# urbste/pyTheiaSfM

Measured on AMD Instinct MI355X. Metric: BA residuals/sec (LM-iterations/sec x observations); RANSAC hypotheses/sec alongside, higher is better.
Workload: dtype f64; 1 GPU; synth_ba_v1 C4: 1000 views / 500000 tracks / 3001239 observations, mixed pinhole + double-sphere (8 intrinsics groups), TRIVIAL loss, intrinsics NONE, homogeneous-manifold points, 8 LM iterations per solve, use_inner_iterations = false on the GPU and the CPU leg (the trust-region step of north_star alone; the reference's default = true is measured in "with_inner_iterations"); views=1000, tracks=500000, observations=3001239, reduced_system_n=6000, k3_levels=8, fused_kernel_runs=2102, n_ranks_seen_by_rccl=1, n_ranks_in_process_group=1

## Files before the change

### pytheiasfm_amd/csrc/ba_fused.hip

```cpp
#define THIP_LEAN_SQRT 1
#define THIP_LEAN_SINCOS 1
#include "ba_fused_lin.h"

#include <algorithm>
#include <cstdio>
#include <cstdlib>

namespace thip {
namespace {

constexpr int kRowBytes = 24;
static_assert(kFusedMaxCams <= kRowBytes, "slot-table row too short");

__global__ __launch_bounds__(256) void k_cam_prep(DevProblem P, const double* __restrict__ cam, const double* __restrict__ intr,
                                                  double* __restrict__ camrot, const double* __restrict__ ycam) {
  const int c = blockIdx.x * blockDim.x + threadIdx.x;
  if (c == 0 && P.frun_next) { P.frun_next[0] = 0; P.frun_next[1] = 0; }
  if (c >= P.nc) return;
  cam_prep_one(P, c, cam + 6 * (size_t)c, intr, camrot);
  if (ycam && P.camdir) {
    const int rc = P.cam_red[c];
    const unsigned mask = P.cam_mask[c];
    double dl[6], ext[6], out[12];
    for (int q = 0; q < 6; ++q)
// ... 199 lines not shown
    double eh[2 * PD];
#pragma unroll
    for (int i = 0; i < 2; ++i)
#pragma unroll
      for (int b = 0; b < PD; ++b) {
        double sm = 0.0;
#pragma unroll
        for (int k = 0; k <= b; ++k) sm += Jt[i * PD + k] * Li[b][k];
        eh[i * PD + b] = sm;
      }
    double2* Rr = reinterpret_cast<double2*>(s_rec + slot * RD);
#pragma unroll
    for (int k = 0; k < 6; ++k) Rr[k] = make_double2(Jc[2 * k], Jc[2 * k + 1]);
#pragma unroll
    for (int k = 0; k < PD; ++k) Rr[6 + k] = make_double2(eh[2 * k], eh[2 * k + 1]);
    Rr[6 + PD] = make_double2(r[0], r[1]);
    double v1[2];
#pragma unroll
    for (int i = 0; i < 2; ++i) {
      double sm = 0.0;
#pragma unroll
      for (int b = 0; b < PD; ++b) sm += eh[i * PD + b] * gh[b];
      v1[i] = r[i] - sm;
    }
    Rr[6 + PD + 1] = make_double2(v1[0], v1[1]);
    s_tslot[c.tl * kRowBytes + c.lc] = (uint8_t)slot;
  }
  sl.lap(stamps, 5);
  const double costw = wave_sum_all(cost);
  gmax = wave_max_all(gmax);
  const double inval = wave_count(active && !valid);
  const double npd = wave_count(active && !pd_ok && sg.head);
  if (lane == 0 && tile_ok) {
    tile_part[4 * (size_t)tile + 0] = costw;
    tile_part[4 * (size_t)tile + 1] = gmax;
    tile_part[4 * (size_t)tile + 2] = inval;
    tile_part[4 * (size_t)tile + 3] = npd;
  }
  sl.lap(stamps, 6);
}

template <int PD, int TPS, unsigned MODELS, int LOSSK, bool STAMPS = false, bool FIRST = false>
__global__ __launch_bounds__(64 * TPS, THIP_FUSED_WAVES) void k_lin_schur(DevProblem P, const double* __restrict__ pts,
                                                           const double* __restrict__ radius_p,
                                                           double* __restrict__ Vinv, double* __restrict__ tile_part,
                                                           double* __restrict__ scale_out = nullptr) {
  constexpr int RD = rec_doubles<PD>();
  constexpr int SUB = TPS * kWave;
  constexpr int SUBT = TPS * kFusedTileTracks;
  constexpr int NWV = TPS;
  __shared__ __attribute__((aligned(16))) double s_rec[SUB * RD];
  __shared__ __attribute__((aligned(16))) double s_cam[kFusedMaxStage * kCamLds];
  __shared__ uint8_t s_tslot[SUBT * kRowBytes];
  __shared__ unsigned s_tmask[SUBT];
  static_assert(SUB * 18 <= SUB * RD, "slice-combination scratch does not fit the record buffer");
  const int tid = threadIdx.x, lane = tid & 63, wv = __builtin_amdgcn_readfirstlane(tid >> 6);
  const double radius = *radius_p;
  const double inv_radius = 1.0 / radius;
  __shared__ int s_next;
  unsigned long long stamps[12];
#pragma unroll
  for (int k = 0; k < 12; ++k) stamps[k] = 0;
  Stamp<STAMPS> sk;
  sk.start();
  int pending = 0;
  if (tid == 0) pending = atomicAdd(P.frun_next, 1);
  for (;;) {
  __syncthreads();
  if (tid == 0) s_next = pending;
  __syncthreads();
  const int rix = __builtin_amdgcn_readfirstlane(s_next);
  if (rix >= P.n_fruns) break;
  if (tid == 0) pending = atomicAdd(P.frun_next, 1);
  const FusedRun run = P.fruns[P.frun_order[rix]];
  const int nsc = (run.ntiles + TPS - 1) / TPS;
  for (int j = tid; j < run.nstage * (kCamRot / 2); j += SUB) {
    const int k = j / (kCamRot / 2), piece = j - k * (kCamRot / 2);
    const int cidx = P.frun_stage[run.stage_off + k];
    reinterpret_cast<double2*>(s_cam + k * kCamLds)[piece] = reinterpret_cast<const double2*>(P.camrot + (size_t)kCamRot * cidx)[piece];
  }
  LanePre<PD> cur;
  int tile = 0; bool tile_ok = false;
  pre_level1<PD, TPS>(P, run, 0, wv, lane, tile, tile_ok, cur);
  pre_level2<PD>(P, pts, cur);
  __syncthreads();

  const int G = run.gp & 0xff, PS = run.gp >> 8;
  int tix, t0, tstride;
  bool slice_ok = true;
  const int B = 64 / PS;
  if (G == 1) { const int g = lane / B; tix = lane - g * B; slice_ok = g < PS; t0 = wv * PS + g; tstride = NWV * PS; }
  else { tix = (wv % G) * 64 + lane; t0 = wv / G; tstride = NWV / G; }
  const bool has_tgt = slice_ok && tix < run.ntgt;
  int la = 0, lb = 0;
  if (has_tgt) { const unsigned us = P.frun_tgt[run.tgt_off + tix]; la = us & 0xffu; lb = us >> 8; }
  const int dix = (G == 1) ? lane : tix;
  const bool has_d = dix < 6 * run.W;
  const int dlc = has_d ? dix / 6 : 0, da = dix % 6;
  const int dP = (G == 1) ? PS : 1, dbase = (G == 1) ? wv * PS : wv / G;
  const unsigned tbits = has_tgt ? ((1u << la) | (1u << lb)) : 0xffffffffu;
  const unsigned dbit = has_d ? (1u << dlc) : 0x80000000u;
  const double diag_core = (has_tgt && la == lb) ? 1.0 : 0.0;
  double acc[36], dacc[3];
#pragma unroll
  for (int k = 0; k < 36; ++k) acc[k] = 0.0;
#pragma unroll
  for (int k = 0; k < 3; ++k) dacc[k] = 0.0;

  sk.lap(stamps, 0);
  for (int sc = 0; sc < nsc; ++sc) {
    LanePre<PD> nxt;
    int ntile = 0; bool ntile_ok = false;
    const int scn = min(sc + 1, nsc - 1);
    pre_level1<PD, TPS>(P, run, scn, wv, lane, ntile, ntile_ok, nxt);
    if (P.fused_dbg & 16) __builtin_amdgcn_s_setprio(1);
    fused_phase_l5<PD, MODELS, LOSSK, STAMPS, FIRST>(P, cur, s_cam, run.W, tile, tile_ok, wv, lane, inv_radius, Vinv, tile_part, s_rec, s_tslot, s_tmask, stamps, scale_out);
    sk.lap(stamps, 1);
    pre_level2<PD>(P, pts, nxt);
    if (P.fused_dbg & 16) __builtin_amdgcn_s_setprio(0);
    if (!(P.fused_dbg & 32)) __builtin_amdgcn_s_setprio(1);
    __syncthreads();
    sk.lap(stamps, 7);
    if (!(P.fused_dbg & 1)) {
      const int last_tile = min(run.tile0 + TPS * sc + TPS - 1, run.tile0 + run.ntiles - 1);
      const int ntr = P.tile_trk_end[last_tile];
      fused_phase_s<PD, RD>(s_rec, s_tslot, s_tmask, ntr, tstride, t0, slice_ok, tbits, la, lb, diag_core, dP, dbase, dbit, dlc, da, acc, dacc);
    }
    sk.lap(stamps, 8);
    if (!(P.fused_dbg & 32)) __builtin_amdgcn_s_setprio(0);
    __syncthreads();
    sk.lap(stamps, 9);
    if constexpr (STAMPS) stamps[11] += 1;
    cur = nxt; tile = ntile; tile_ok = ntile_ok;
  }
  double* scratch = s_rec;
  double* out = P.fpart + run.part_off;
  const int nrep = (G == 1) ? NWV * PS : NWV / G;
#pragma unroll
  for (int h = 0; h < 2; ++h) {
    if (h) __syncthreads();
#pragma unroll
    for (int q = 0; q < 18; ++q) scratch[tid * 18 + q] = acc[18 * h + q];
    __syncthreads();
    for (int e = tid; e < run.ntgt * 18; e += SUB) {
      const int k = e / 18, q = e - 18 * k;
      double v = scratch[k * 18 + q];
#pragma unroll 1
      for (int r = 1; r < nrep; ++r) {
        const int oth = (G == 1) ? ((r / PS) * 64 + (r % PS) * B + k) : (k + r * G * 64);
        v += scratch[oth * 18 + q];
      }
      out[(size_t)k * 36 + 18 * h + q] = v;
    }
  }
  __syncthreads();
#pragma unroll
  for (int q = 0; q < 3; ++q) scratch[tid * 3 + q] = dacc[q];
  __syncthreads();
  if (has_d && tid == dix) {
    const int nrd = (G == 1) ? NWV : NWV / G;
    double v[3];
#pragma unroll
    for (int q = 0; q < 3; ++q) v[q] = scratch[tid * 3 + q];
#pragma unroll 1
    for (int r = 1; r < nrd; ++r) {
      const int oth = (G == 1) ? (r * 64 + dix) : (dix + r * G * 64);
#pragma unroll
      for (int q = 0; q < 3; ++q) v[q] += scratch[oth * 3 + q];
    }
    double* od = out + (size_t)run.ntgt * 36 + (size_t)dix * 3;
#pragma unroll
    for (int q = 0; q < 3; ++q) od[q] = v[q];
  }
  sk.lap(stamps, 10);
  }
  if constexpr (STAMPS) {
    if (lane == 0) {
#pragma unroll
      for (int k = 0; k < 12; ++k) atomicAdd(&g_fused_stamps[k], stamps[k]);
    }
  }
}

constexpr int kCamLdsB = 70;

constexpr int kCamLdsBI = 82;
template <int PD, int TPS, unsigned MODELS, int LOSSK, int WPS, bool INTR = false, unsigned KMASK = 0u>
__global__ __launch_bounds__(64 * TPS, WPS) void k_backsub_runs(DevProblem P, const double* __restrict__ pts, double* __restrict__ cand_pts,
                                                             const double* __restrict__ Vinv, double* __restrict__ tile_part,
                                                             const double* __restrict__ ysol = nullptr) {
  constexpr int NT = PD * (PD + 1) / 2;
  constexpr int SUB = TPS * kWave;
  constexpr int PITCH = INTR ? kCamLdsBI : kCamLdsB;
  constexpr int OFF_CAND = INTR ? 56 : 52;
  constexpr int OFF_CINTR = INTR ? 72 : kCamRotIntr;
  __shared__ __attribute__((aligned(16))) double s_cam[(INTR ? kFusedMaxStageIntr : kFusedMaxStage) * PITCH];
  __shared__ __attribute__((aligned(16))) double s_slot[TPS][64 * 4];
  __shared__ int s_next;
  const int tid = threadIdx.x, lane = tid & 63, wv = __builtin_amdgcn_readfirstlane(tid >> 6);
  int pending = 0;
  if (tid == 0) pending = atomicAdd(P.frun_next + 1, 1);
  for (;;) {
  __syncthreads();
// ... 443 lines not shown
```

### pytheiasfm_amd/csrc/ba_kernels.h

```cpp
#pragma once
#include <algorithm>
#include <vector>
#include <hip/hip_runtime.h>
#include <cstdint>

#include "dense_cholesky.h"

namespace thip {

struct FusedRun {
  int tile0, ntiles;
  int cam_off, W;
  int tgt_off, ntgt;
  int part_off;
  int gp;
  int stage_off, nstage;
};
inline int fused_tiles_per_subchunk(int) { return 4; }
constexpr int kFusedMaxCams = 22;
constexpr int kFusedMaxConst = 22;
constexpr int kFusedMaxStage = kFusedMaxCams + kFusedMaxConst;
constexpr int kFusedTileTracks = 32;
constexpr int kFusedIntrRows = 4, kFusedIntrWidth = 6 + kFusedIntrRows;
constexpr int kFusedMaxCamsIntr = 12;
constexpr int kFusedMaxConstIntr = 12;
constexpr int kFusedMaxStageIntr = kFusedMaxCamsIntr + kFusedMaxConstIntr;

struct DevProblem {
  int nc, np, ncv, ntiles;
  int64_t nobs;
  int n;
  int pd;
  int loss_type;
  double loss_width;
  const double* intr;
  const int* group_model;
  const int* cam_group;
  const int* cam_red;
  const uint8_t* cam_mask;
  const uint8_t* pt_const;
  const double2* obs_uv;
  const double2* obs_si;
  const int* obs_cam;
  const int* obs_pt;
  const int* tile_start;
  const int* tile_count;
  int long_nobs, long_ntracks;
  const int* long_obs_index;
  const int* long_obs_slot;
  const int* long_track_start;
  const int* long_track_pt;
  const double* scale_c;
  const double* scale_p;
  int ni;
  int ng_total;
  const int* grp_k;
  const int* grp_red;
  const unsigned* grp_free;
  const unsigned* red_free;
// ... 228 lines not shown
```

### pytheiasfm_amd/csrc/ba_plan.hip

```cpp
#include <atomic>
#include <cstdio>
#include <limits>
#include <map>
#include <mutex>
#include <new>

#include "ba_handle.h"
#include "ba_host_rules.h"

namespace {

template <class T>
struct NoInitAlloc : std::allocator<T> {
  template <class U> struct rebind { using other = NoInitAlloc<U>; };
  template <class U, class... A>
  void construct(U* ptr, A&&... args) {
    if constexpr (sizeof...(A) == 0) ::new (static_cast<void*>(ptr)) U; else ::new (static_cast<void*>(ptr)) U(std::forward<A>(args)...);
  }
};

template <class T>
struct RawArray {
  std::unique_ptr<T[]> p;
  explicit RawArray(size_t n) : p(new T[std::max<size_t>(1, n)]) {}
  T& operator[](size_t i) { return p[i]; }
  const T& operator[](size_t i) const { return p[i]; }
  T* data() { return p.get(); }
};

template <class T, class Digit>
void counting_pass(const T* from, T* to, int64_t n, int nb, Digit&& digit) {
  int parts = host_part_count(n, 32768);
  if (n < 393216 && !getenv("THEIA_HIP_HOST_CHUNK_MIN")) parts = 1;
  if ((int64_t)parts * nb > ((int64_t)1 << 24)) parts = 1;
  const int64_t per = (n + parts - 1) / parts;
  std::vector<int> head((size_t)parts * nb, 0);
  host_parts(parts, true, [&](int t) {
    int* hh = head.data() + (size_t)t * nb;
    for (int64_t i = t * per; i < std::min<int64_t>(n, (t + 1) * per); ++i) hh[digit(from[i])]++;
  });
  int run = 0;
  for (int b = 0; b < nb; ++b)
    for (int t = 0; t < parts; ++t) { int& c = head[(size_t)t * nb + b]; const int cnt = c; c = run; run += cnt; }
  host_parts(parts, true, [&](int t) {
    int* hh = head.data() + (size_t)t * nb;
    for (int64_t i = t * per; i < std::min<int64_t>(n, (t + 1) * per); ++i) to[hh[digit(from[i])]++] = from[i];
  });
}

__global__ void k_fill_value(double* x, size_t n, double v) {
  for (size_t i = (size_t)blockIdx.x * blockDim.x + threadIdx.x; i < n; i += (size_t)gridDim.x * blockDim.x) x[i] = v;
}

const int kCfgF2S[3][8] = {{SC_COST, SC_GMAX, SC_INVALID, SC_NOTPD, 0, 0, 0, 0},
                           {SB_COST, SB_MCC, SB_STEPSQ, SB_XNORMSQ, SB_INVALID, 0, 0, 0},
                           {SB_COST, SB_INVALID, 0, 0, 0, 0, 0, 0}};
const int kCfgMax[3][8] = {{0, 1, 0, 0, 0, 0, 0, 0}, {0, 0, 0, 0, 0, 0, 0, 0}, {0, 0, 0, 0, 0, 0, 0, 0}};

#define UP(buf, vec) do { rc = h->buf.upload(vec, st); if (rc) return rc; } while (0)
#define AL(buf, cnt) do { rc = h->buf.alloc(cnt); if (rc) return rc; } while (0)
int build_gather_lists(theia_ba_handle_s* h, const int* ocam, const int* opt,
// ... 331 lines not shown
  const bool compact = h->intr_rows == 4;
  emit_pairs(gg, [&](int ga, int gb, int64_t beg, int64_t end) {
    push_item(IT_GG0, 10 * ga, 10 * gb, beg, end, 1 | (ga == gb ? 2 : 0));
    if (!compact) push_item(IT_GG1, 10 * ga, 10 * gb, beg, end, 1 | (ga == gb ? 2 : 0));
  });
  itick("sorted pair lists");
  if (npairs > (size_t)std::numeric_limits<int>::max() - 64)
    return set_error(THEIA_HIP_ERR_UNSUPPORTED, "too many observation pairs for 32-bit pair lists");
  for (size_t q = 0; q < order.size();) {
    size_t e = q + 1;
    while (e < order.size() && red[order[e]] == red[order[q]] && grd[order[e]] == grd[order[q]]) ++e;
    const int rc = red[order[q]], gr = grd[order[q]];
    if (rc >= 0) {
      push_item(IT_CD, h->ni + 6 * rc, h->ni + 6 * rc, (int64_t)q, (int64_t)e, self[rc] ? 1 : 0);
      if (gr >= 0) push_item(IT_CGD, h->ni + 6 * rc, 10 * gr, (int64_t)q, (int64_t)e, 1);
    }
    q = e;
  }
  for (size_t q = 0; q < order.size();) {
    size_t e = q + 1;
    while (e < order.size() && grd[order[e]] == grd[order[q]]) ++e;
    const int gr = grd[order[q]];
    if (gr >= 0) {
      push_item(IT_GD0, 10 * gr, 10 * gr, (int64_t)q, (int64_t)e, 1);
      if (!compact) push_item(IT_GD1, 10 * gr, 10 * gr, (int64_t)q, (int64_t)e, 1);
      push_item(IT_GV, 10 * gr, 10 * gr, (int64_t)q, (int64_t)e, 0);
    }
    q = e;
  }
  h->n_diag_items = 0; h->n_blk_items = (int)items.size() / 6;
  {
    std::vector<int> sobs(order.begin(), order.end());
    if (sobs.empty()) sobs.push_back(0);
    UP(slot_obs, sobs);
  }
  UP(cam_obs, slot); UP(blk_items, items);
  if ((rc = h->blk_pairs.upload(pairs.data(), std::max<size_t>(1, npairs), st, pairs.pinned()))) return rc;
  itick("items + uploads");
  h->n_trk_sums = nsums;
  h->sum_base = nslots;
  if (nsums) { UP(pt_sum_slot, pt_sum); UP(slot_in_sum, slot_sum); UP(pt_sum_cnt, pt_cnt); UP(sum_group, sum_group); }
  AL(rec, (std::max<size_t>(1, order.size()) + (size_t)h->n_trk_sums) * (12 * h->pd + 20 + 2 * h->intr_rows * h->pd + 3 * h->intr_rows));
  return 0;
}

inline int fused_run_cameras(int bw) {
  if (bw == 0) return kFusedMaxCams;
  if (bw == 9) return kFusedMaxCamsIntr;
  if (bw == 10) return 10;
  return 10;
}
inline int fused_lanes_per_target(int bw) { return bw == 0 ? 1 : (bw <= 10 ? (bw + 2) / 3 : (bw + 3) / 4); }

struct FusedHost {
  std::vector<FusedRun> runs;
  std::vector<int> cams, stage, tile_trk_end, sum_items, sum_src;
  std::vector<unsigned short> tgts;
  std::vector<uint8_t> obs_lc, obs_tl;
  std::vector<uint8_t> tile_adj;
  size_t part_doubles = 0;
};
struct FusedSegment {
  std::vector<int> tstart, tcount, tkey, l_obs, l_slot, l_start, l_pt;
  FusedHost fp;
};
void build_fused_segment(const theia_ba_handle_s* h, const std::vector<int64_t>& off, const std::vector<int>& porder,
                         const int* sred, const int* ocam, const std::vector<int>& skey, int q_begin, int q_end,
                         uint8_t* obs_lc, uint8_t* obs_tl, FusedSegment& seg) {
  std::vector<int>& tstart = seg.tstart; std::vector<int>& tcount = seg.tcount; std::vector<int>& tkey = seg.tkey;
  std::vector<int>& l_obs = seg.l_obs; std::vector<int>& l_slot = seg.l_slot; std::vector<int>& l_start = seg.l_start;
  std::vector<int>& l_pt = seg.l_pt;
  FusedHost& fp = seg.fp;
  const int64_t nm = h->nobs_main;
  const int tps = fused_tiles_per_subchunk(h->pd);
  const int bw = h->fused_bw;
  const size_t lanes_tgt = bw == 0 ? 1 : (size_t)fused_lanes_per_target(bw), rows_cam = bw == 0 ? 6 : (size_t)bw;
  const size_t part_tgt = bw == 0 ? 36 : (size_t)bw * bw, part_cam = bw == 0 ? 18 : (size_t)3 * bw;
  const int max_cams = fused_run_cameras(bw);
  const size_t max_tgts = bw == 0 ? 253 : 256 / lanes_tgt;
  auto packing = [&](size_t ntgt, size_t W) -> int {
    if (lanes_tgt * ntgt > 64 || rows_cam * W > 64) return 0;
    static const int cand[6] = {10, 6, 4, 3, 2, 1};
    for (int c : cand) if ((size_t)(64 / c) >= lanes_tgt * ntgt) return c;
    return 1;
  };
  const char* rm = getenv("THEIA_HIP_FUSED_RUN_OBS");
  const int64_t run_max = rm ? std::max(64, atoi(rm)) : std::max<int64_t>(256, std::min<int64_t>(2048, nm / 600));
  int64_t t_start = 0, t_len = 0;
  int t_tracks = 0, sc_tracks = 0;
  int run_tile0 = 0, run_ntiles = 0, run_key0 = -1;
  int64_t run_obs = 0;
  std::vector<int> run_cams;
  std::vector<int64_t> run_pairs;
  std::vector<int> tc;
  std::vector<int64_t> tp;
  int serial = 1, prev_serial = 0;
  std::vector<int> prev_tc;
  std::vector<int> cam_stamp((size_t)std::max(1, h->ncp), 0);
  std::vector<uint8_t> cam_local((size_t)std::max(1, h->ncp), 0);
  const int max_const = bw == 0 ? kFusedMaxConst : kFusedMaxConstIntr;
  static_assert(kFusedMaxConst <= 0x7f && kFusedMaxConstIntr <= 0x7f, "obs_lc keeps the constant-camera index in seven bits");
  std::vector<int> run_ccams, tcc;
  std::vector<int> ccam_stamp((size_t)std::max(1, h->nc), 0);
  std::vector<uint8_t> ccam_local((size_t)std::max(1, h->nc), 0);
  constexpr int kPairSlots = 2048;
  std::vector<int64_t> pair_key(kPairSlots, 0);
  std::vector<int> pair_stamp(kPairSlots, 0);
  auto pair_slot = [&](int64_t key) -> int {
    unsigned hsh = ((unsigned)(key >> 32) * 0x9E3779B1u) ^ ((unsigned)key * 0x85EBCA77u);
    int sl = (int)(hsh >> 21) & (kPairSlots - 1);
    while (pair_stamp[sl] == serial && pair_key[sl] != key) sl = (sl + 1) & (kPairSlots - 1);
    return sl;
  };
  const int adj_nt = (h->n + 63) / 64;
  fp.tile_adj.assign((size_t)adj_nt * adj_nt, 0);
  std::vector<int> tl;
  auto mark_tiles = [&](int q) {
    if (h->pt_const[porder[q]]) return;
    tl.clear();
    for (int pcam : tc) {
      const int rcam = h->cam_red[h->part_cam[pcam]];
      if (rcam < 0) continue;
      const int s0 = h->ni + 6 * rcam;
      if (tl.empty() || tl.back() != s0 / 64) tl.push_back(s0 / 64);
      if ((s0 + 5) / 64 != s0 / 64) tl.push_back((s0 + 5) / 64);
    }
    for (int a : tl) for (int b : tl) fp.tile_adj[(size_t)a * adj_nt + b] = 1;
  };

  auto close_tile = [&](int q_end) {
    if (!t_len) return;
    tstart.push_back((int)t_start); tcount.push_back((int)t_len); tkey.push_back(run_key0 < 0 ? 0 : run_key0);
    (void)q_end;
    fp.tile_trk_end.push_back(sc_tracks);
    run_ntiles++;
    t_len = 0; t_tracks = 0;
  };
  auto finalize_run = [&]() {
    if (!run_ntiles) { run_cams.clear(); run_pairs.clear(); run_ccams.clear(); run_obs = 0; run_key0 = -1; ++serial; return; }
    std::sort(run_cams.begin(), run_cams.end());
    std::sort(run_pairs.begin(), run_pairs.end());
    FusedRun r;
    r.tile0 = run_tile0; r.ntiles = run_ntiles;
    r.cam_off = (int)fp.cams.size(); r.W = (int)run_cams.size();
    fp.cams.insert(fp.cams.end(), run_cams.begin(), run_cams.end());
    r.tgt_off = (int)fp.tgts.size(); r.ntgt = (int)run_pairs.size();
    for (size_t i = 0; i < run_cams.size(); ++i) cam_local[run_cams[i]] = (uint8_t)i;
    for (int64_t key : run_pairs) {
      const int la = cam_local[(int)(key >> 32)], lb = cam_local[(int)(key & 0xffffffff)];
      fp.tgts.push_back((unsigned short)(la | (lb << 8)));
    }
    const int need = (int)std::max(lanes_tgt * r.ntgt, rows_cam * r.W);
    const int G = need <= 64 ? 1 : (need <= 128 ? 2 : 4);
    r.gp = G | ((G == 1 ? std::max(1, packing((size_t)r.ntgt, (size_t)r.W)) : 1) << 8);
    r.part_off = (int)fp.part_doubles;
    fp.part_doubles += (size_t)r.ntgt * part_tgt + (size_t)r.W * part_cam;
    r.stage_off = (int)fp.stage.size();
    for (int pc : run_cams) fp.stage.push_back(h->part_cam[pc]);
    fp.stage.insert(fp.stage.end(), run_ccams.begin(), run_ccams.end());
    r.nstage = (int)(run_cams.size() + run_ccams.size());
    for (int t = run_tile0; t < run_tile0 + run_ntiles; ++t)
      for (int s = tstart[t]; s < tstart[t] + tcount[t]; ++s) {
        if (sred[s] >= 0) obs_lc[s] = cam_local[sred[s]];
        else obs_lc[s] = (uint8_t)(0x80 | ccam_local[ocam[s]]);
      }
    fp.runs.push_back(r);
    run_tile0 += run_ntiles; run_ntiles = 0; run_obs = 0; run_key0 = -1;
    run_cams.clear(); run_pairs.clear(); run_ccams.clear(); ++serial;
  };
  auto push_long = [&](int q) {
    const int slot = (int)l_pt.size();
    l_pt.push_back(porder[q]);
    for (int64_t c = off[q]; c < off[q + 1]; ++c) { l_obs.push_back((int)c); l_slot.push_back(slot); }
    l_start.push_back((int)l_obs.size());
  };
  run_tile0 = (int)tstart.size();
  for (int q = q_begin; q < q_end; ++q) {
    const int64_t L = off[q + 1] - off[q];
    if (L == 0) continue;
    tc.clear(); tcc.clear();
    for (int64_t s = off[q]; s < off[q + 1]; ++s) {
      if (sred[s] >= 0) tc.push_back(sred[s]);
      else tcc.push_back(ocam[s]);
    }
    std::sort(tc.begin(), tc.end());
    const bool dup = std::adjacent_find(tc.begin(), tc.end()) != tc.end();
    if (!tcc.empty()) { std::sort(tcc.begin(), tcc.end()); tcc.erase(std::unique(tcc.begin(), tcc.end()), tcc.end()); }
    mark_tiles(q);
    if (L > 64 || dup || (int)tc.size() > max_cams || (int)tcc.size() > max_const) {
      close_tile(q);
      push_long(q);
      continue;
    }
    const bool same_set = serial == prev_serial && tc == prev_tc;
    size_t ucams = run_cams.size(), upairs = run_pairs.size();
    if (!same_set) {
      tp.clear();
      for (size_t a = 0; a < tc.size(); ++a)
        for (size_t b = 0; b <= a; ++b) tp.push_back(((int64_t)tc[a] << 32) | (uint32_t)tc[b]);
      for (int c : tc) ucams += cam_stamp[c] != serial;
      for (int64_t key : tp) upairs += pair_stamp[pair_slot(key)] != serial;
    }
    bool new_run = (int)ucams > max_cams || upairs > max_tgts;
    if (!tcc.empty()) {
      size_t uc = run_ccams.size();
      for (int c : tcc) uc += ccam_stamp[c] != serial;
      if (uc > (size_t)max_const) new_run = true;
    }
    auto level = [&](size_t ntgt, size_t W) -> int {
      const int pk = packing(ntgt, W);
      if (bw == 0 || pk > 0) return bw == 0 ? pk : 4;
      const size_t need = std::max(lanes_tgt * ntgt, rows_cam * W);
      return need <= 128 ? 2 : 1;
    };
    if (!new_run && run_obs >= 64 && level(upairs, ucams) < level(run_pairs.size(), run_cams.size())) new_run = true;
    if (!new_run && run_obs >= run_max / 4 && skey[q] != run_key0) new_run = true;
    if (new_run) {
      close_tile(q);
      finalize_run();
    }
    if (t_len + L > 64 || t_tracks >= kFusedTileTracks) {
      close_tile(q);
      const size_t need = std::max(lanes_tgt * run_pairs.size(), rows_cam * run_cams.size());
      const int64_t cap = bw ? run_max : (need <= 64 ? run_max : (need <= 128 ? run_max / 4 : 1));
      if (run_ntiles % tps == 0 && run_obs >= cap) finalize_run();
    }
    if (t_len == 0) {
      t_start = off[q];
      if (run_ntiles % tps == 0) sc_tracks = 0;
      if (run_key0 < 0) run_key0 = skey[q];
    }
    for (int64_t s = off[q]; s < off[q + 1]; ++s) obs_tl[s] = (uint8_t)sc_tracks;
    sc_tracks++; t_tracks++; t_len += L; run_obs += L;
    if (!(same_set && serial == prev_serial)) {
      if (same_set) {
        tp.clear();
        for (size_t a = 0; a < tc.size(); ++a)
          for (size_t b = 0; b <= a; ++b) tp.push_back(((int64_t)tc[a] << 32) | (uint32_t)tc[b]);
      }
      for (int c : tc) if (cam_stamp[c] != serial) { cam_stamp[c] = serial; run_cams.push_back(c); }
      for (int64_t key : tp) {
        const int sl = pair_slot(key);
        if (pair_stamp[sl] != serial) { pair_stamp[sl] = serial; pair_key[sl] = key; run_pairs.push_back(key); }
      }
      prev_tc = tc; prev_serial = serial;
    }
    for (int c : tcc) if (ccam_stamp[c] != serial) { ccam_stamp[c] = serial; ccam_local[c] = (uint8_t)run_ccams.size(); run_ccams.push_back(c); }
  }
  close_tile(q_end);
  finalize_run();
}

int build_sum_items_intr(theia_ba_handle_s* h, const int* cam_group, FusedHost& fp, int* n_items1, int* n_items2) {
  constexpr int SK_BLOCK = 0, SK_LOWER = 1, SK_VEC = 2, SK_CHUNK = 3;
  const int KI = h->fused_bw - 6, ni = h->ni, BW = h->fused_bw;
  struct Ent { int64_t key; int off, code, dims; };
  auto src_code = [](int r0, int c0, int tr, int stride) { return r0 | (c0 << 4) | (tr << 8) | (stride << 16); };
  auto dims = [](int nr, int nc, int kind, int rg, int cg) { return nr | (nc << 4) | (kind << 8) | (rg << 12) | (cg << 13); };
  auto key_blk = [](int row0, int col0) { return ((int64_t)row0 << 30) | (int64_t)col0; };
  auto key_vec = [](int row0) { return ((int64_t)1 << 60) | ((int64_t)row0 << 30); };
  constexpr int kRunParts = 32;
  const int nruns = (int)fp.runs.size();
  auto emit = [&](int ir, auto&& sink) {
    const FusedRun& r = fp.runs[ir];
    auto cam_of = [&](int l) { return h->part_cam[fp.cams[r.cam_off + l]]; };
    for (int k = 0; k < r.ntgt; ++k) {
      const unsigned us = fp.tgts[r.tgt_off + k];
      const int la = us & 0xff, lb = us >> 8;
      const int ca = cam_of(la), cb = cam_of(lb);
      const int rca = h->cam_red[ca], rcb = h->cam_red[cb], ga = h->grp_red[cam_group[ca]], gb = h->grp_red[cam_group[cb]];
      const int base = r.part_off + BW * BW * k;
      if (rca >= 0 && rcb >= 0)
        sink(Ent{key_blk(ni + 6 * rca, ni + 6 * rcb), base, src_code(0, 0, 0, BW), dims(6, 6, la == lb ? SK_LOWER : SK_BLOCK, 0, 0)});
      if (rca >= 0 && gb >= 0)
        sink(Ent{key_blk(ni + 6 * rca, 10 * gb), base, src_code(0, 6, 0, BW), dims(6, KI, SK_BLOCK, 0, 1)});
      if (la != lb && rcb >= 0 && ga >= 0)
        sink(Ent{key_blk(ni + 6 * rcb, 10 * ga), base, src_code(6, 0, 1, BW), dims(6, KI, SK_BLOCK, 0, 1)});
      if (ga >= 0 && gb >= 0) {
        const int nh = KI > 7 ? 2 : 1, hr = KI > 7 ? KI / 2 : KI;
        for (int hh = 0; hh < nh; ++hh) {
          const int r0 = hh * hr, nr = (hh == nh - 1) ? KI - r0 : hr;
          if (ga > gb) sink(Ent{key_blk(10 * ga + r0, 10 * gb), base, src_code(6 + r0, 6, 0, BW), dims(nr, KI, SK_BLOCK, 1, 1)});
          else if (ga < gb) sink(Ent{key_blk(10 * gb + r0, 10 * ga), base, src_code(6, 6 + r0, 1, BW), dims(nr, KI, SK_BLOCK, 1, 1)});
          else {
            sink(Ent{key_blk(10 * ga + r0, 10 * ga), base, src_code(6 + r0, 6, 0, BW), dims(nr, KI, SK_LOWER, 1, 1)});
            if (la != lb) sink(Ent{key_blk(10 * ga + r0, 10 * ga), base, src_code(6, 6 + r0, 1, BW), dims(nr, KI, SK_LOWER, 1, 1)});
          }
        }
      }
    }
    for (int l = 0; l < r.W; ++l) {
      const int c = cam_of(l), rc = h->cam_red[c], gr = h->grp_red[cam_group[c]];
      const int base = r.part_off + BW * BW * r.ntgt + 3 * BW * l;
      if (rc >= 0) sink(Ent{key_vec(ni + 6 * rc), base, src_code(0, 0, 0, 3), dims(6, 3, SK_VEC, 0, 0)});
      if (gr >= 0) sink(Ent{key_vec(10 * gr), base, src_code(6, 0, 0, 3), dims(KI, 3, SK_VEC, 1, 0)});
    }
  };
  std::vector<size_t> at(kRunParts + 1, 0);
  host_parts(kRunParts, nruns >= 256, [&](int part) {
    size_t cnt = 0;
// ... 597 lines not shown
    for (int64_t i = 0; i < h->nobs; ++i)
      if (h->cam_red[p->obs_cam[i]] >= 0 && !h->pt_const[p->obs_pt[i]]) off[p->obs_pt[i] + 1]++;
    for (int q = 0; q < h->np; ++q) off[q + 1] += off[q];
    std::vector<int> rcs(off[h->np]);
    {
      std::vector<int64_t> fill(off.begin(), off.end() - 1);
      for (int64_t i = 0; i < h->nobs; ++i) {
        const int rcam = h->cam_red[p->obs_cam[i]];
        if (rcam >= 0 && !h->pt_const[p->obs_pt[i]]) rcs[fill[p->obs_pt[i]]++] = rcam;
      }
    }
    std::vector<int> tl;
    for (int q = 0; q < h->np; ++q) {
      tl.clear();
      for (int64_t k = off[q]; k < off[q + 1]; ++k) {
        const int s0 = h->ni + 6 * rcs[k];
        tl.push_back(s0 / 64);
        if ((s0 + 5) / 64 != s0 / 64) tl.push_back((s0 + 5) / 64);
      }
      std::sort(tl.begin(), tl.end());
      tl.erase(std::unique(tl.begin(), tl.end()), tl.end());
      for (int a : tl) for (int b : tl) h->tile_adj[(size_t)a * nt + b] = 1;
    }
    }
    for (int rcam = 0; rcam < h->ncv; ++rcam) {
      const int s0 = h->ni + 6 * rcam, a = s0 / 64, b = (s0 + 5) / 64;
      h->tile_adj[(size_t)a * nt + a] = 1;
      h->tile_adj[(size_t)b * nt + b] = 1;
      h->tile_adj[(size_t)a * nt + b] = h->tile_adj[(size_t)b * nt + a] = 1;
    }
    h->tile_touch.assign(nt, 0);
    for (int c = 0; c < h->nc; ++c) {
      const bool prior = p->cam_prior_mask && o->prior_mask && (p->cam_prior_mask[c] & o->prior_mask);
      if ((!cam_used[c] && !prior) || h->cam_red[c] < 0) continue;
      const int s0 = h->ni + 6 * h->cam_red[c];
      h->tile_touch[s0 / 64] = 1; h->tile_touch[(s0 + 5) / 64] = 1;
    }
    for (int a = 0; a < (h->ni + 63) / 64; ++a)
      for (int b = 0; b < nt; ++b) h->tile_adj[(size_t)a * nt + b] = h->tile_adj[(size_t)b * nt + a] = 1;
    tick("priors + tile adjacency");
    h->plan = chol_plan_create(h->n, h->tile_adj.data());
    tick("K3 plan");
  }
  if (h->ni == 0 && h->ntiles_main > 0 && (rc = build_gather_lists(h, ocam, opt, l_obs, !h->use_fused))) return rc;
  if (h->use_fused) {
    h->n_fruns = (int)fplan.runs.size(); h->n_sum_items = (int)fplan.sum_items.size() / 6 - h->n_sum_items2;
    fplan.tile_trk_end.resize(std::max<size_t>(1, fplan.tile_trk_end.size()));
    if (ctiming) {
      std::map<int, std::pair<int, int>> by;
      long long nsc = 0;
      for (const FusedRun& r : fplan.runs) { auto& e = by[r.gp]; e.first++; e.second += (r.ntiles + 3) / 4; nsc += (r.ntiles + 3) / 4; }
      fprintf(stderr, "theia_hip fused plan: %zu runs, %lld sub-chunks (%.1f obs each), %zu partial doubles, %d sum items\n",
              fplan.runs.size(), nsc, nsc ? (double)h->nobs_main / nsc : 0.0, fplan.part_doubles, h->n_sum_items);
      for (auto& kv : by) fprintf(stderr, "  G=%d slices/wave=%d: %d runs, %d sub-chunks\n", kv.first & 0xff, kv.first >> 8, kv.second.first, kv.second.second);
    }
    if (fplan.runs.empty()) fplan.runs.push_back(FusedRun{0, 0, 0, 0, 0, 0, 0, 1 | (1 << 8), 0, 0});
    {
      std::vector<int> order(fplan.runs.size());
      for (size_t i = 0; i < order.size(); ++i) order[i] = (int)i;
      const int lanes_tgt = fused_lanes_per_target(h->fused_bw);
      auto cost = [&](int i) { const FusedRun& r = fplan.runs[i]; return (long long)r.ntiles * (64 + lanes_tgt * r.ntgt); };
      std::stable_sort(order.begin(), order.end(), [&](int a, int b) { return cost(a) > cost(b); });
      UP(frun_order, order);
      AL(frun_next, 2);
    }
    fplan.stage.resize(std::max<size_t>(1, fplan.stage.size()));
    UP(fruns, fplan.runs); UP(frun_cams, fplan.cams); UP(frun_stage, fplan.stage); UP(frun_tgt, fplan.tgts); UP(obs_lc, fplan.obs_lc); UP(obs_tl, fplan.obs_tl);
    UP(tile_trk_end, fplan.tile_trk_end); UP(sum_items, fplan.sum_items); UP(sum_src, fplan.sum_src);
    AL(fpart, std::max<size_t>(1, fplan.part_doubles));
    AL(camrot, (size_t)40 * std::max(1, h->nc)); AL(camrot_cand, (size_t)40 * std::max(1, h->nc)); AL(camdir, (size_t)12 * std::max(1, h->nc));
  }
  if (h->ni > 0 && !h->use_fused && h->ntiles_main > 0 && (rc = build_gather_lists_intr(h, p, ocam, opt, l_obs))) return rc;
#undef UP
#undef AL
  tick("gather lists");
  fill_devproblem(h);
  rc = upload_parameters(h, p);
  if (rc) return rc;
  tick("parameter upload");
  double fc = 0.0, inv = 0.0;
  rc = cost_of_tiles(h, h->ntiles_eval, h->ntiles_all - h->ntiles_eval, h->cam[0].p, h->pts[0].p, &fc, &inv);
  if (rc) return rc;
  if (h->n_priors) {
    double pf = 0.0;
    HIP_TRYR(hipMemsetAsync(h->scalB.p, 0, sizeof(double) * 16, h->stream));
    launch_cam_priors(h->P, PRIOR_FIXED, h->cam[0].p, nullptr, nullptr, nullptr, nullptr, h->scalB.p, nullptr, h->stream);
    HIP_TRYR(hipStreamSynchronize(h->stream));
    HIP_TRYR(hipMemcpy(&pf, h->scalB.p, sizeof(double), hipMemcpyDeviceToHost));
    fc += pf;
  }
  h->fixed_cost = fc;
  tick("fixed cost");
  *out = guard.release();
  return 0;
}

}

extern "C" int theia_hip_ba_create(const theia_ba_problem* p, const theia_ba_options* o, theia_ba_handle* out) {
  debug_sticky("create entry");
  int rc = ba_create_impl(p, o, out, true);
  if (rc == kRetryWithoutFusedIntr) rc = ba_create_impl(p, o, out, false);
  debug_sticky("create exit");
  return rc;
}
```

Measured before the change: 3.835 billion residuals/s.

## Deal tracks into unequal-width lane slices in fused Schur phase

The planner now sizes per-wave lane slices to each track's target need (the last camera's diagonal index), instead of splitting 64 lanes into equal slices. It also deals tracks into slots so sub-chunks need fewer rows, and keeps the layout only when it saves at least about 1/16 of the rows. The kernel reads a per-run slice table, double-buffers the track mask so each buffer is cleared after a barrier, and reduces partials across the unequal slices. A hashed seen-set cache replaces the single previous-set check, and an optional plan-occupancy JSON dump is added. The changes add planning complexity and some runtime branching in the kernel.

After: 3.883 billion residuals/s, median of 6. 1.3% higher.

```diff
diff --git a/pytheiasfm_amd/csrc/ba_fused.hip b/pytheiasfm_amd/csrc/ba_fused.hip
--- a/pytheiasfm_amd/csrc/ba_fused.hip
+++ b/pytheiasfm_amd/csrc/ba_fused.hip
@@ -275,8 +275,10 @@
   __shared__ __attribute__((aligned(16))) double s_rec[SUB * RD];
   __shared__ __attribute__((aligned(16))) double s_cam[kFusedMaxStage * kCamLds];
   __shared__ uint8_t s_tslot[SUBT * kRowBytes];
-  __shared__ unsigned s_tmask[SUBT];
+  __shared__ unsigned s_tmask[2 * SUBT];
+  __shared__ unsigned short s_slice[16];
   static_assert(SUB * 18 <= SUB * RD, "slice-combination scratch does not fit the record buffer");
+  static_assert(kFusedMaxSlices <= 16, "slice table too short");
   const int tid = threadIdx.x, lane = tid & 63, wv = __builtin_amdgcn_readfirstlane(tid >> 6);
   const double radius = *radius_p;
   const double inv_radius = 1.0 / radius;
@@ -288,6 +290,7 @@
   sk.start();
   int pending = 0;
   if (tid == 0) pending = atomicAdd(P.frun_next, 1);
+  for (int j = tid; j < 2 * SUBT; j += SUB) s_tmask[j] = 0u;
   for (;;) {
   __syncthreads();
   if (tid == 0) s_next = pending;
@@ -308,11 +311,22 @@
   pre_level2<PD>(P, pts, cur);
   __syncthreads();
 
-  const int G = run.gp & 0xff, PS = run.gp >> 8;
+  const int G = run.gp & 0xff, PS = (run.gp >> 8) & 0xff;
+  const bool unequal = (run.gp & kFusedUnequalSlices) != 0;
   int tix, t0, tstride;
   bool slice_ok = true;
   const int B = 64 / PS;
-  if (G == 1) { const int g = lane / B; tix = lane - g * B; slice_ok = g < PS; t0 = wv * PS + g; tstride = NWV * PS; }
+  if (unequal) {
+    int g = 0, at = 0;
+    slice_ok = false;
+    for (int j = 0; j < PS; ++j) {
+      const int us = P.frun_tgt[run.tgt_off + run.ntgt + j], oj = us & 0xff, wj = us >> 8;
+      if (lane >= oj && lane < oj + wj) { g = j; at = oj; slice_ok = true; }
+      if (tid == j) s_slice[j] = (unsigned short)us;
+    }
+    tix = lane - at; t0 = wv * PS + g; tstride = NWV * PS;
+  }
+  else if (G == 1) { const int g = lane / B; tix = lane - g * B; slice_ok = g < PS; t0 = wv * PS + g; tstride = NWV * PS; }
   else { tix = (wv % G) * 64 + lane; t0 = wv / G; tstride = NWV / G; }
   const bool has_tgt = slice_ok && tix < run.ntgt;
   int la = 0, lb = 0;
@@ -337,7 +351,8 @@
     const int scn = min(sc + 1, nsc - 1);
     pre_level1<PD, TPS>(P, run, scn, wv, lane, ntile, ntile_ok, nxt);
     if (P.fused_dbg & 16) __builtin_amdgcn_s_setprio(1);
-    fused_phase_l5<PD, MODELS, LOSSK, STAMPS, FIRST>(P, cur, s_cam, run.W, tile, tile_ok, wv, lane, inv_radius, Vinv, tile_part, s_rec, s_tslot, s_tmask, stamps, scale_out);
+    unsigned* const tmask = s_tmask + (sc & 1) * SUBT;
+    fused_phase_l5<PD, MODELS, LOSSK, STAMPS, FIRST>(P, cur, s_cam, run.W, tile, tile_ok, wv, lane, inv_radius, Vinv, tile_part, s_rec, s_tslot, tmask, stamps, scale_out);
     sk.lap(stamps, 1);
     pre_level2<PD>(P, pts, nxt);
     if (P.fused_dbg & 16) __builtin_amdgcn_s_setprio(0);
@@ -347,11 +362,12 @@
     if (!(P.fused_dbg & 1)) {
       const int last_tile = min(run.tile0 + TPS * sc + TPS - 1, run.tile0 + run.ntiles - 1);
       const int ntr = P.tile_trk_end[last_tile];
-      fused_phase_s<PD, RD>(s_rec, s_tslot, s_tmask, ntr, tstride, t0, slice_ok, tbits, la, lb, diag_core, dP, dbase, dbit, dlc, da, acc, dacc);
+      fused_phase_s<PD, RD>(s_rec, s_tslot, tmask, ntr, tstride, t0, slice_ok, tbits, la, lb, diag_core, dP, dbase, dbit, dlc, da, acc, dacc);
     }
     sk.lap(stamps, 8);
     if (!(P.fused_dbg & 32)) __builtin_amdgcn_s_setprio(0);
     __syncthreads();
+    if (tid < SUBT) tmask[tid] = 0u;
     sk.lap(stamps, 9);
     if constexpr (STAMPS) stamps[11] += 1;
     cur = nxt; tile = ntile; tile_ok = ntile_ok;
@@ -368,10 +384,20 @@
     for (int e = tid; e < run.ntgt * 18; e += SUB) {
       const int k = e / 18, q = e - 18 * k;
       double v = scratch[k * 18 + q];
+      if (unequal) {
+#pragma unroll 1
+        for (int j = 0; j < PS; ++j) {
+          const int us = s_slice[j], oj = us & 0xff, wj = us >> 8;
+          if (k >= wj) break;
+#pragma unroll 1
+          for (int w = (j == 0) ? 1 : 0; w < NWV; ++w) v += scratch[(w * 64 + oj + k) * 18 + q];
+        }
+      } else {
 #pragma unroll 1
       for (int r = 1; r < nrep; ++r) {
         const int oth = (G == 1) ? ((r / PS) * 64 + (r % PS) * B + k) : (k + r * G * 64);
         v += scratch[oth * 18 + q];
+      }
       }
       out[(size_t)k * 36 + 18 * h + q] = v;
     }
diff --git a/pytheiasfm_amd/csrc/ba_fused_slices.h b/pytheiasfm_amd/csrc/ba_fused_slices.h
--- /dev/null
+++ b/pytheiasfm_amd/csrc/ba_fused_slices.h
@@ -0,0 +1,8 @@
+#pragma once
+
+namespace thip {
+
+constexpr int kFusedUnequalSlices = 1 << 16;
+constexpr int kFusedMaxSlices = 10;
+
+}
diff --git a/pytheiasfm_amd/csrc/ba_kernels.h b/pytheiasfm_amd/csrc/ba_kernels.h
--- a/pytheiasfm_amd/csrc/ba_kernels.h
+++ b/pytheiasfm_amd/csrc/ba_kernels.h
@@ -5,6 +5,7 @@
 #include <cstdint>
 
 #include "dense_cholesky.h"
+#include "ba_fused_slices.h"
 
 namespace thip {
 
diff --git a/pytheiasfm_amd/csrc/ba_plan.hip b/pytheiasfm_amd/csrc/ba_plan.hip
--- a/pytheiasfm_amd/csrc/ba_plan.hip
+++ b/pytheiasfm_amd/csrc/ba_plan.hip
@@ -7,6 +7,7 @@
 
 #include "ba_handle.h"
 #include "ba_host_rules.h"
+#include "ba_plan_stats.h"
 
 namespace {
 
@@ -444,6 +445,10 @@
 }
 inline int fused_lanes_per_target(int bw) { return bw == 0 ? 1 : (bw <= 10 ? (bw + 2) / 3 : (bw + 3) / 4); }
 
+constexpr double kFusedRunCostSteps = 64.0;
+
+inline std::atomic<long long>& shape_mismatches() { static std::atomic<long long> n{0}; return n; }
+
 struct FusedHost {
   std::vector<FusedRun> runs;
   std::vector<int> cams, stage, tile_trk_end, sum_items, sum_src;
@@ -486,8 +491,10 @@
   std::vector<int64_t> run_pairs;
   std::vector<int> tc;
   std::vector<int64_t> tp;
-  int serial = 1, prev_serial = 0;
-  std::vector<int> prev_tc;
+  int serial = 1;
+  struct SeenSet { int stamp = 0, n = 0; int cams[kFusedMaxCams]; };
+  constexpr int kSeenSets = 64;
+  std::vector<SeenSet> seen_sets(kSeenSets);
   std::vector<int> cam_stamp((size_t)std::max(1, h->ncp), 0);
   std::vector<uint8_t> cam_local((size_t)std::max(1, h->ncp), 0);
   const int max_const = bw == 0 ? kFusedMaxConst : kFusedMaxConstIntr;
@@ -528,8 +535,105 @@
     run_ntiles++;
     t_len = 0; t_tracks = 0;
   };
+  struct RunTrack { int s0, cmax, tile; uint8_t len, need; };
+  std::vector<RunTrack> run_trk;
+  int run_kmin = 64;
+  std::vector<int> need_desc, sc_gt, sc_n, sc_first, slot_of, sc_slots, by_need;
+  const bool unequal_slices = !getenv("THEIA_HIP_FUSED_EQUAL_SLICES");
+  auto shape_slices = [&](FusedRun& r) {
+    const int PS0 = r.gp >> 8, ntrk = (int)run_trk.size(), nsc = (run_ntiles + tps - 1) / tps;
+    if (r.ntgt < 2 || ntrk < 8 || r.ntgt + std::max(1, run_kmin * (run_kmin + 1) / 2) > 64) return;
+    int hist[66] = {0}, diag_at[kFusedMaxCams] = {0};
+    for (int k = 0; k < r.ntgt; ++k) { const unsigned us = fp.tgts[(size_t)r.tgt_off + k]; if ((us & 0xff) == (us >> 8)) diag_at[us & 0xff] = k + 1; }
+    int least = 64;
+    for (RunTrack& t : run_trk) { t.need = (uint8_t)(t.cmax >= 0 ? diag_at[cam_local[t.cmax]] : 0); hist[t.need]++; least = std::min<int>(least, t.need); }
+    if (r.ntgt + std::max(1, least) > 64) return;
+    const size_t NW = (size_t)r.ntgt + 1;
+    need_desc.clear();
+    for (int v = 64; v >= 0; --v) need_desc.insert(need_desc.end(), (size_t)hist[v], v);
+    sc_gt.assign((size_t)nsc * NW, 0); sc_n.assign((size_t)nsc, 0); sc_first.assign((size_t)nsc + 1, ntrk);
+    for (int i = ntrk - 1; i >= 0; --i) {
+      const int sc = (run_trk[i].tile - run_tile0) / tps;
+      sc_first[sc] = i; sc_n[sc]++;
+      if (run_trk[i].need > 0) sc_gt[(size_t)sc * NW + run_trk[i].need - 1]++;
+    }
+    for (int sc = 0; sc < nsc; ++sc)
+      for (int v = r.ntgt - 2; v >= 0; --v) sc_gt[(size_t)sc * NW + v] += sc_gt[(size_t)sc * NW + v + 1];
+    for (int sc = nsc - 1; sc >= 0; --sc) if (sc_n[sc] == 0) sc_first[sc] = sc_first[sc + 1];
+    auto rows_of = [&](const int* wid, int p) -> long long {
+      long long rows = 0;
+      for (int sc = 0; sc < nsc; ++sc) {
+        int rs = (sc_n[sc] + p - 1) / p;
+        for (int j = 1; j < p; ++j) {
+          const int over = sc_gt[(size_t)sc * NW + wid[j]];
+          if (!over) continue;
+          int wider = 0;
+          while (wider < j && wid[wider] > wid[j]) ++wider;
+          rs = std::max(rs, (over + wider - 1) / std::max(1, wider));
+        }
+        if (rs * p > kFusedTileTracks * tps) return -1;
+        rows += rs;
+      }
+      return rows;
+    };
+    int eq[kFusedMaxSlices];
+    for (int j = 0; j < PS0; ++j) eq[j] = r.ntgt;
+    const long long rows_eq = rows_of(eq, PS0);
+    int best[kFusedMaxSlices], bestp = 0, last[kFusedMaxSlices], lastp = 0, tried = 0;
+    long long best_rows = -1;
+    for (int R = (ntrk + kFusedMaxSlices - 1) / kFusedMaxSlices; R < ntrk && tried < 2; ++R) {
+      int wid[kFusedMaxSlices], p = 0, sum = 0;
+      for (int j = 0; j * R < ntrk && p < kFusedMaxSlices && sum <= 64; ++j) {
+        const int w = j == 0 ? r.ntgt : need_desc[(size_t)j * R];
+        if (w == 0) break;
+        wid[p++] = w; sum += w;
+      }
+      if (sum > 64 || p < 2) continue;
+      if (p == lastp && std::equal(wid, wid + p, last)) continue;
+      std::copy(wid, wid + p, last); lastp = p; ++tried;
+      for (int variant = 0; variant < 2; ++variant) {
+        if (variant)
+          for (int j = p - 1; j >= 1; --j) {
+            int up = wid[j] + 1;
+            while (up <= wid[j - 1] && !hist[up]) ++up;
+            if (up <= wid[j - 1] && sum - wid[j] + up <= 64) { sum += up - wid[j]; wid[j] = up; }
+          }
+        const long long rows = rows_of(wid, p);
+        if (rows >= 0 && (best_rows < 0 || rows < best_rows)) { best_rows = rows; bestp = p; std::copy(wid, wid + p, best); }
+      }
+    }
+    if (best_rows < 0 || rows_eq < 0 || best_rows * 16 > rows_eq * 15) return;
+    slot_of.assign((size_t)ntrk, 0); sc_slots.assign((size_t)nsc, 0);
+    uint8_t fits_of[66];
+    for (int v = 0, fits = bestp; v <= r.ntgt; ++v) { while (fits > 0 && best[fits - 1] < v) --fits; fits_of[v] = (uint8_t)fits; }
+    long long dealt_rows = 0;
+    for (int sc = 0; sc < nsc; ++sc) {
+      {
+        int at[66];
+        for (int v = 0; v <= r.ntgt; ++v) at[v] = sc_gt[(size_t)sc * NW + v];
+        by_need.assign((size_t)(sc_first[sc + 1] - sc_first[sc]), 0);
+        for (int i = sc_first[sc]; i < sc_first[sc + 1]; ++i) by_need[(size_t)at[run_trk[i].need]++] = i;
+      }
+      int fill[kFusedMaxSlices] = {0};
+      for (int i : by_need) {
+        const int fits = fits_of[run_trk[i].need];
+        int to = 0;
+        for (int j = 1; j < fits; ++j) if (fill[j] <= fill[to]) to = j;
+        const int slot = fill[to]++ * bestp + to;
+        if (slot >= kFusedTileTracks * tps) return;
+        slot_of[i] = slot; sc_slots[sc] = std::max(sc_slots[sc], slot + 1);
+      }
+      dealt_rows += *std::max_element(fill, fill + bestp);
+    }
+    if (dealt_rows != best_rows) { shape_mismatches().fetch_add(1, std::memory_order_relaxed); return; }
+    for (int i = 0; i < ntrk; ++i)
+      for (int s = run_trk[i].s0; s < run_trk[i].s0 + run_trk[i].len; ++s) obs_tl[s] = (uint8_t)slot_of[i];
+    for (int sc = 0; sc < nsc; ++sc) fp.tile_trk_end[(size_t)run_tile0 + std::min(run_ntiles, (sc + 1) * tps) - 1] = sc_slots[sc];
+    r.gp = 1 | (bestp << 8) | kFusedUnequalSlices;
+    for (int j = 0, at = 0; j < bestp; ++j) { fp.tgts.push_back((unsigned short)(at | (best[j] << 8))); at += best[j]; }
+  };
   auto finalize_run = [&]() {
-    if (!run_ntiles) { run_cams.clear(); run_pairs.clear(); run_ccams.clear(); run_obs = 0; run_key0 = -1; ++serial; return; }
+    if (!run_ntiles) { run_cams.clear(); run_pairs.clear(); run_ccams.clear(); run_trk.clear(); run_kmin = 64; run_obs = 0; run_key0 = -1; ++serial; return; }
     std::sort(run_cams.begin(), run_cams.end());
     std::sort(run_pairs.begin(), run_pairs.end());
     FusedRun r;
@@ -545,6 +649,7 @@
     const int need = (int)std::max(lanes_tgt * r.ntgt, rows_cam * r.W);
     const int G = need <= 64 ? 1 : (need <= 128 ? 2 : 4);
     r.gp = G | ((G == 1 ? std::max(1, packing((size_t)r.ntgt, (size_t)r.W)) : 1) << 8);
+    if (bw == 0 && G == 1 && unequal_slices) shape_slices(r);
     r.part_off = (int)fp.part_doubles;
     fp.part_doubles += (size_t)r.ntgt * part_tgt + (size_t)r.W * part_cam;
     r.stage_off = (int)fp.stage.size();
@@ -558,7 +663,7 @@
       }
     fp.runs.push_back(r);
     run_tile0 += run_ntiles; run_ntiles = 0; run_obs = 0; run_key0 = -1;
-    run_cams.clear(); run_pairs.clear(); run_ccams.clear(); ++serial;
+    run_cams.clear(); run_pairs.clear(); run_ccams.clear(); run_trk.clear(); run_kmin = 64; ++serial;
   };
   auto push_long = [&](int q) {
     const int slot = (int)l_pt.size();
@@ -584,7 +689,11 @@
       push_long(q);
       continue;
     }
-    const bool same_set = serial == prev_serial && tc == prev_tc;
+    unsigned set_hash = (unsigned)tc.size();
+    for (int c : tc) set_hash = set_hash * 0x9E3779B1u + (unsigned)c;
+    SeenSet& seen = seen_sets[(set_hash >> 16) & (kSeenSets - 1)];
+    const int prev_serial = serial;
+    const bool same_set = seen.stamp == serial && seen.n == (int)tc.size() && std::equal(tc.begin(), tc.end(), seen.cams);
     size_t ucams = run_cams.size(), upairs = run_pairs.size();
     if (!same_set) {
       tp.clear();
@@ -635,9 +744,12 @@
         const int sl = pair_slot(key);
         if (pair_stamp[sl] != serial) { pair_stamp[sl] = serial; pair_key[sl] = key; run_pairs.push_back(key); }
       }
-      prev_tc = tc; prev_serial = serial;
+      seen.stamp = serial; seen.n = (int)tc.size();
+      std::copy(tc.begin(), tc.end(), seen.cams);
     }
     for (int c : tcc) if (ccam_stamp[c] != serial) { ccam_stamp[c] = serial; ccam_local[c] = (uint8_t)run_ccams.size(); run_ccams.push_back(c); }
+    run_trk.push_back(RunTrack{(int)off[q], tc.empty() ? -1 : tc.back(), (int)tstart.size(), (uint8_t)L, 0});
+    run_kmin = std::min(run_kmin, (int)tc.size());
   }
   close_tile(q_end);
   finalize_run();
@@ -1341,7 +1453,15 @@
       for (const FusedRun& r : fplan.runs) { auto& e = by[r.gp]; e.first++; e.second += (r.ntiles + 3) / 4; nsc += (r.ntiles + 3) / 4; }
       fprintf(stderr, "theia_hip fused plan: %zu runs, %lld sub-chunks (%.1f obs each), %zu partial doubles, %d sum items\n",
               fplan.runs.size(), nsc, nsc ? (double)h->nobs_main / nsc : 0.0, fplan.part_doubles, h->n_sum_items);
-      for (auto& kv : by) fprintf(stderr, "  G=%d slices/wave=%d: %d runs, %d sub-chunks\n", kv.first & 0xff, kv.first >> 8, kv.second.first, kv.second.second);
+      fprintf(stderr, "  slice shapes whose dealing missed the closed-form rows (process total): %lld\n", shape_mismatches().load());
+      for (auto& kv : by) fprintf(stderr, "  G=%d slices/wave=%d%s: %d runs, %d sub-chunks\n", kv.first & 0xff, (kv.first >> 8) & 0xff, (kv.first & kFusedUnequalSlices) ? " (unequal)" : "", kv.second.first, kv.second.second);
+    }
+    if (const char* sp = getenv("THEIA_HIP_PLAN_STATS")) {
+      if (*sp && h->fused_bw == 0) {
+        const PlanStats ps = fused_plan_occupancy(fplan.runs.data(), (int)fplan.runs.size(), fplan.tgts.data(), tstart.data(), tcount.data(),
+                                                  fplan.tile_trk_end.data(), fplan.obs_lc.data(), fplan.obs_tl.data(), fused_tiles_per_subchunk(h->pd));
+        if (FILE* f = fopen(sp, "w")) { write_plan_stats_json(f, ps, kFusedRunCostSteps); fclose(f); }
+      }
     }
     if (fplan.runs.empty()) fplan.runs.push_back(FusedRun{0, 0, 0, 0, 0, 0, 0, 1 | (1 << 8), 0, 0});
     {
diff --git a/pytheiasfm_amd/csrc/ba_plan_stats.h b/pytheiasfm_amd/csrc/ba_plan_stats.h
--- /dev/null
+++ b/pytheiasfm_amd/csrc/ba_plan_stats.h
@@ -0,0 +1,131 @@
+#pragma once
+#include <algorithm>
+#include <cstdint>
+#include <cstdio>
+#include <vector>
+
+#include "ba_fused_slices.h"
+
+namespace thip {
+
+struct PlanRunStats {
+  int ntgt = 0, W = 0, G = 1, PS = 1, unequal = 0, tiles = 0, obs = 0, tracks = 0;
+  long long steps = 0, skipped = 0;
+  long long useful = 0;
+  long long idle_shape = 0;
+  long long idle_sparsity = 0;
+  void add(const PlanRunStats& o) {
+    tiles += o.tiles; obs += o.obs; tracks += o.tracks; steps += o.steps; skipped += o.skipped;
+    useful += o.useful; idle_shape += o.idle_shape; idle_sparsity += o.idle_sparsity;
+  }
+};
+struct PlanStats {
+  std::vector<PlanRunStats> runs;
+  PlanRunStats total;
+};
+
+inline int fused_run_slices(int gp, int ntgt, const unsigned short* after_targets, int (&off)[kFusedMaxSlices], int (&wid)[kFusedMaxSlices]) {
+  const int PS = std::min(kFusedMaxSlices, std::max(1, (gp >> 8) & 0xff));
+  for (int g = 0; g < PS; ++g) {
+    if (gp & kFusedUnequalSlices) { off[g] = after_targets[g] & 0xff; wid[g] = after_targets[g] >> 8; }
+    else { off[g] = g * (64 / PS); wid[g] = std::min(64 / PS, ntgt); }
+  }
+  return PS;
+}
+
+template <class Run>
+PlanStats fused_plan_occupancy(const Run* runs, int nruns, const unsigned short* tgts, const int* tile_start, const int* tile_count,
+                               const int* tile_trk_end, const uint8_t* obs_lc, const uint8_t* obs_tl, int tps, int nwv = 4) {
+  PlanStats out;
+  out.runs.resize((size_t)std::max(0, nruns));
+  std::vector<unsigned> mask, filled;
+  std::vector<unsigned> tb;
+  for (int ir = 0; ir < nruns; ++ir) {
+    const Run& r = runs[ir];
+    PlanRunStats& st = out.runs[ir];
+    st.ntgt = r.ntgt; st.W = r.W; st.G = r.gp & 0xff; st.PS = std::max(1, (r.gp >> 8) & 0xff); st.unequal = (r.gp & kFusedUnequalSlices) ? 1 : 0;
+    st.tiles = r.ntiles;
+    tb.assign((size_t)r.ntgt, 0u);
+    for (int k = 0; k < r.ntgt; ++k) { const unsigned us = tgts[r.tgt_off + k]; tb[k] = (1u << (us & 0xff)) | (1u << (us >> 8)); }
+    int off[kFusedMaxSlices], wid[kFusedMaxSlices];
+    const int G = st.G, PS = G == 1 ? fused_run_slices(r.gp, r.ntgt, tgts + r.tgt_off + r.ntgt, off, wid) : 1;
+    int lanes_in_slices = 0;
+    for (int g = 0; g < PS && G == 1; ++g) lanes_in_slices += st.unequal ? wid[g] : 64 / PS;
+    for (int t0 = 0; t0 < r.ntiles; t0 += tps) {
+      const int t1 = std::min(r.ntiles, t0 + tps);
+      const int ntr = tile_trk_end[r.tile0 + t1 - 1];
+      mask.assign((size_t)std::max(1, ntr), 0u); filled.assign((size_t)std::max(1, ntr), 0u);
+      for (int t = r.tile0 + t0; t < r.tile0 + t1; ++t)
+        for (int s = tile_start[t]; s < tile_start[t] + tile_count[t]; ++s) {
+          st.obs++;
+          if (obs_tl[s] >= ntr) continue;
+          if (!filled[obs_tl[s]]) { filled[obs_tl[s]] = 1u; st.tracks++; }
+          if (!(obs_lc[s] & 0x80)) mask[obs_tl[s]] |= 1u << obs_lc[s];
+        }
+      auto have = [&](int t, int k0, int k1, long long* hit, long long* miss) {
+        for (int k = k0; k < k1; ++k) { if ((mask[t] & tb[k]) == tb[k]) ++*hit; else ++*miss; }
+      };
+      const int tstride = G == 1 ? nwv * PS : std::max(1, nwv / G);
+      for (int wv = 0; wv < nwv; ++wv)
+        for (int base = 0; base < ntr; base += tstride) {
+          long long hit = 0, miss = 0, shape = 0;
+          if (G == 1) {
+            shape = 64 - lanes_in_slices;
+            for (int g = 0; g < PS; ++g) {
+              const int t = base + wv * PS + g, lanes = st.unequal ? wid[g] : 64 / PS;
+              if (t < ntr && filled[t]) { have(t, 0, wid[g], &hit, &miss); shape += lanes - wid[g]; }
+              else shape += lanes;
+            }
+          } else {
+            const int t = base + wv / G, k0 = std::min(r.ntgt, 64 * (wv % G)), k1 = std::min(r.ntgt, k0 + 64);
+            if (t < ntr && filled[t]) { have(t, k0, k1, &hit, &miss); shape = 64 - (k1 - k0); }
+            else shape = 64;
+          }
+          if (hit) { st.steps++; st.useful += hit; st.idle_sparsity += miss; st.idle_shape += shape; }
+          else st.skipped++;
+        }
+    }
+    out.total.add(st);
+  }
+  return out;
+}
+
+inline void write_plan_stats_json(FILE* f, const PlanStats& ps, double run_cost_steps) {
+  auto frac = [](long long a, long long b) { return b ? (double)a / (double)b : 0.0; };
+  auto body = [&](const PlanRunStats& s) {
+    fprintf(f, "\"tiles\": %d, \"observations\": %d, \"tracks\": %d, \"steps_issued\": %lld, \"steps_skipped\": %lld, \"lanes_issued\": %lld, "
+            "\"lanes_useful\": %lld, \"lanes_idle_shape\": %lld, \"lanes_idle_sparsity\": %lld, \"lane_efficiency\": %.4f, "
+            "\"share_idle_shape\": %.4f, \"share_idle_sparsity\": %.4f",
+            s.tiles, s.obs, s.tracks, s.steps, s.skipped, 64 * s.steps, s.useful, s.idle_shape, s.idle_sparsity, frac(s.useful, 64 * s.steps),
+            frac(s.idle_shape, 64 * s.steps), frac(s.idle_sparsity, 64 * s.steps));
+  };
+  fprintf(f, "{\n \"model\": \"phase S of k_lin_schur: wave steps that run the FMA body x 64 lanes against (track, target) items\",\n");
+  fprintf(f, " \"runs\": %zu, \"run_cost_steps\": %.1f, \"objective_steps\": %.1f,\n \"total\": {", ps.runs.size(), run_cost_steps,
+          (double)ps.total.steps + run_cost_steps * (double)ps.runs.size());
+  body(ps.total);
+  fprintf(f, "},\n \"by_shape\": [");
+  std::vector<std::pair<int, PlanRunStats>> by;
+  std::vector<int> nby;
+  for (const PlanRunStats& s : ps.runs) {
+    const int key = s.G | (s.PS << 8) | (s.unequal << 16);
+    size_t k = 0;
+    while (k < by.size() && by[k].first != key) ++k;
+    if (k == by.size()) { by.push_back({key, PlanRunStats()}); nby.push_back(0); by[k].second.G = s.G; by[k].second.PS = s.PS; by[k].second.unequal = s.unequal; }
+    by[k].second.add(s); nby[k]++;
+  }
+  for (size_t k = 0; k < by.size(); ++k) {
+    fprintf(f, "%s\n  {\"G\": %d, \"PS\": %d, \"unequal_slices\": %d, \"runs\": %d, ", k ? "," : "", by[k].second.G, by[k].second.PS, by[k].second.unequal, nby[k]);
+    body(by[k].second);
+    fprintf(f, "}");
+  }
+  fprintf(f, "\n ],\n \"run_columns\": [\"ntgt\", \"W\", \"G\", \"PS\", \"unequal_slices\", \"tiles\", \"observations\", \"tracks\", \"steps_issued\", \"steps_skipped\", "
+          "\"lanes_useful\", \"lanes_idle_shape\", \"lanes_idle_sparsity\"],\n \"run_rows\": [");
+  for (size_t k = 0; k < ps.runs.size(); ++k) {
+    const PlanRunStats& s = ps.runs[k];
+    fprintf(f, "%s\n  [%d, %d, %d, %d, %d, %d, %d, %d, %lld, %lld, %lld, %lld, %lld]", k ? "," : "", s.ntgt, s.W, s.G, s.PS, s.unequal, s.tiles, s.obs, s.tracks,
+            s.steps, s.skipped, s.useful, s.idle_shape, s.idle_sparsity);
+  }
+  fprintf(f, "\n ]\n}\n");
+}
+
+}
```
